# bibendovsky/oalsfxpp

Hardware: AMD Instinct MI355X
Metric: Msamples/sec EAX reverb, 256-frame buffers, batch=4096; % HBM roofline (higher is better)
Workload: dtype f32

## Files before the change

include/oalsfx_hip_debug.h:

```cpp
#ifndef OALSFX_HIP_DEBUG_H
#define OALSFX_HIP_DEBUG_H

#include "oalsfx_hip.h"

#ifdef __cplusplus
extern "C" {
#endif

int oalsfx_batch_mix_timed(oalsfx_batch* b, int frames, const float* src_host, float* dst_host, double legs_us[3]);
long long oalsfx_debug_chain_same_cu(oalsfx_batch* b);
int oalsfx_batch_fill_synthetic(oalsfx_batch* b, int frames, unsigned buffer_index, float* dst_dev, void* hip_stream);

int oalsfx_batch_kernel_timing(oalsfx_batch* b, int enable);
int oalsfx_batch_kernel_timing_read(oalsfx_batch* b, int effect_type, int* launches, double* total_ms);
int oalsfx_batch_kernel_timing_samples(oalsfx_batch* b, int effect_type, double* out_us, int max_samples);
int oalsfx_batch_placement(const oalsfx_batch* b, int* chunks, int* candidates, double* best_us, double* worst_us);
int oalsfx_batch_event_overhead(oalsfx_batch* b, int repeats, double* avg_us);

int oalsfx_debug_hbm_sweep(int device_id, unsigned long long bytes, int write, int repeats);
void oalsfx_debug_set_flags(int flags);
unsigned long long oalsfx_debug_ring_address(oalsfx_batch* b, int instance, int slot);
int oalsfx_debug_move_rings(oalsfx_batch* b, int keep_old);
int oalsfx_debug_probe_rings(oalsfx_batch* b, int repeats, double* avg_us);
int oalsfx_debug_probe_pointer(void* slabs, int instances, int slab_floats, int repeats, double* avg_us);
int oalsfx_debug_stream_pattern(int device_id, int instances, int dwords_per_lane, int repeats, int slab_floats, int pos_skew, double* avg_us);

int oalsfx_debug_host_pipeline(oalsfx_batch* b, int* form, double* probe_us_three_streams, double* probe_us_one_stream);

void oalsfx_debug_gate_skew(oalsfx_batch* b, unsigned skew);
int oalsfx_debug_chain_given_up(const oalsfx_batch* b);
int oalsfx_debug_chain_started(oalsfx_batch* b, unsigned* host_total, unsigned* device_total);
int oalsfx_batch_multi_counts(const oalsfx_batch* b, long long* buffers_in_passes, long long* passes);

long long oalsfx_debug_downmix_uploads(const oalsfx_batch* b);
void oalsfx_debug_downmix_vector(int max_floats);

long long oalsfx_debug_sampler_uploads(const oalsfx_batch* b);
long long oalsfx_debug_envelope_uploads(const oalsfx_batch* b);
const char* oalsfx_debug_last_render_kernel(const oalsfx_batch* b);
long long oalsfx_debug_resampler_uploads(const oalsfx_batch* b);

#ifdef __cplusplus
}
#endif

#endif
```

oalsfxpp_amd/api.py:

```python
import ctypes as C
import operator
import weakref

import numpy as np

from . import desc, lib

_fp = C.POINTER(C.c_float)
DOWNMIX_CHUNK = 32
METER_LANES = 64
METER_CARRY = 1
METER_DTYPE = np.dtype([("peak", np.float32, (desc.MAX_CHANNELS,)), ("sumsq", np.float32, (desc.MAX_CHANNELS,)), ("peak_hold", np.float32),
                        ("quiet_run", np.uint32), ("nonfinite", np.uint32), ("frames", np.uint32)])
assert METER_DTYPE.itemsize == C.sizeof(desc.Meter) == 80
SAMPLER_DTYPE = np.dtype([("data", np.uint64), ("position", np.uint64), ("frames", np.uint32), ("loop_start", np.uint32), ("loop_end", np.uint32),
                          ("step", np.uint32), ("format", np.uint32), ("channels", np.uint32), ("flags", np.uint32), ("reserved", np.uint32),
                          ("gain", np.float32, (desc.MAX_CHANNELS,))])
assert SAMPLER_DTYPE.itemsize == C.sizeof(desc.Sampler) == 80
SAMPLER_FRAC_BITS = desc.SAMPLER_FRAC_BITS
ENVELOPE_DTYPE = np.dtype([("flags", np.uint32), ("delay", np.uint32), ("ramp_frames", np.uint32), ("ramp_done", np.uint32),
                           ("gain_from", np.float32, (desc.MAX_CHANNELS,)), ("gain_step", np.float32, (desc.MAX_CHANNELS,)),
                           ("gain_to", np.float32, (desc.MAX_CHANNELS,)), ("glide_frames", np.uint32), ("glide_done", np.uint32),
                           ("glide_slope", np.int32), ("step_to", np.uint32), ("sub", np.uint32), ("reserved", np.uint32, (3,))])
assert ENVELOPE_DTYPE.itemsize == C.sizeof(desc.Envelope) == 144
# ... 175 lines not shown

    def mix_device(self, frames, src_ptr, dst_ptr, stream=None):
        self._check(self._lib.oalsfx_batch_mix_device(self._h, frames, C.c_void_p(src_ptr), C.c_void_p(dst_ptr), C.c_void_p(stream or 0)))

    def mix_device_multi(self, frames, src_ptrs, dst_ptrs, stream=None):
        if len(src_ptrs) != len(dst_ptrs):
            raise BatchError("mix_device_multi: as many source as destination buffers")
        s = (C.c_void_p * max(1, len(src_ptrs)))(*src_ptrs)
        d = (C.c_void_p * max(1, len(dst_ptrs)))(*dst_ptrs)
        self._check(self._lib.oalsfx_batch_mix_device_multi(self._h, frames, len(src_ptrs), s, d, C.c_void_p(stream or 0)))

    def multi_counts(self):
        k, p = C.c_longlong(0), C.c_longlong(0)
        self._check(self._lib.oalsfx_batch_multi_counts(self._h, C.byref(k), C.byref(p)))
        return k.value, p.value

    def synchronize(self):
        self._check(self._lib.oalsfx_batch_synchronize(self._h))

    @property
    def stream(self):
        return self._lib.oalsfx_batch_stream(self._h)

    def fill_synthetic(self, frames, buffer_index, dst_ptr, stream=None):
        self._check(self._lib.oalsfx_batch_fill_synthetic(self._h, frames, buffer_index, C.c_void_p(dst_ptr), C.c_void_p(stream or 0)))

    def read_slot(self, instance, slot):
        p, s = desc.SlotParams(), desc.SlotState()
        self._check(self._lib.oalsfx_batch_read_slot(self._h, instance, slot, C.byref(p), C.byref(s)))
        return p, s
# ... 586 lines not shown
```

oalsfxpp_amd/csrc/hip/batch.cpp:

```cpp
#include <hip/hip_runtime.h>

#include <algorithm>
#include <atomic>
#include <cstdio>
#include <chrono>
#include <cmath>
#include <cstdlib>
#include <cstring>
#include <map>
#include <mutex>
#include <new>
#include <string>
#include <type_traits>
#include <vector>

#include "../host/core.hpp"
#include "common.hpp"
#include "oalsfx_hip.h"
#include "state_io.hpp"
#include "downmix.hpp"
#include "meter.hpp"
#include "sampler.hpp"
#include "voice.hpp"
#include "resample.hpp"
// ... 145 lines not shown
    uint32_t turn_counter = 0;
    uint32_t started_total = 0;
    int launched_groups = 0;
    uint32_t frames_total = 0;
    std::vector<uint32_t> started_at;
    bool off_grid_known = false;
    int off_grid[OALSFX_MAX_SLOTS] = {};
    bool poisoned = false;
    int chain_len = 0;
    std::vector<std::pair<const char*, const char*>> chain_dsts;
    bool uncached = false;
    bool chain_open = false;
    bool stream_handed_out = false;
    long long chained_calls = 0;
    long long multi_buffers = 0, multi_passes = 0;
    std::vector<int> route_bus;
    std::vector<float> route_gain;
    bool routing_dirty = true;
    int route_max = -1;
    int dm_buses = 0;
    oalsfx_hip::DownmixTable dm_table;
    oalsfx_hip::DownmixDevice dm_dev;
    char* h_dm_table = nullptr;
    char* d_dm_table = nullptr;
    size_t dm_table_capacity = 0;
    float* d_dm_partials = nullptr;
    size_t dm_partials_capacity = 0;
    float* d_dm_out = nullptr;
    size_t dm_out_capacity = 0;
    hipEvent_t ev_downmix = nullptr;
// ... 109 lines not shown
        b->ring_floats[idx] = 0;
    }
}

enum DebugFlag : int {
    kDbgAcquireAlways = 0x1,
    kDbgAcquireNever = 0x2,
    kDbgReadEarly = 0x4,
    kDbgGeneralOnly = 0x8,
    kDbgTapRound128 = 0x20,
    kDbgTapRound256 = 0x40,
    kDbgChainLight = 0x80,
    kDbgNoCuMajor = 0x100,
    kDbgNoChain = 0x400,
    kDbgGateSecondOnly = 0x800,
    kDbgChainAlways = 0x8000,
    kDbgForceProven = 0x2000000,
    kDbgHandOverBits = kDbgAcquireAlways | kDbgAcquireNever | kDbgReadEarly,
    kDbgKernelBits = 0xFF,
};
int debug_flags();

constexpr int kSettleFrames = OALSFX_RV_FADE_SAMPLES;

enum : uint8_t {
    kClassReverb = 1,
    kClassSteady = 2,
    kClassClose = 4,
    kClassShort = 8,
    kClassModulated = 16,
// ... 364 lines not shown
        st.capacity = cap;
    }
    return &st;
}

struct PendingUpload {
    bool any = false;
    oalsfx_batch::Stage* st = nullptr;
    size_t bytes = 0;
    bool direct = true;
    bool chainable = true;
    oalsfx_hip::UploadJobs jobs{};
};

bool chain_join(oalsfx_batch* b);

bool prepare_params(oalsfx_batch* b, PendingUpload& pu)
{
    if (b->dirty_list.empty() && !b->lists_dirty) return true;
    pu.any = true;
    const size_t total = static_cast<size_t>(b->n) * b->slots;
    std::map<size_t, int> need;
    std::vector<size_t> restarted;
    std::vector<int> up_params, up_state, up_source, up_touched;
    std::vector<uint32_t> up_epoch;
    bool any_type_change = false;
    if (!b->dirty_list.empty()) b->upload_gen += 1;

    if (b->last_launch_stream && b->last_launch_stream != b->stream) {
        if (!b->hip_ok(hipStreamWaitEvent(b->stream, b->ev_mixed, 0), "hipStreamWaitEvent")) return false;
// ... 500 lines not shown
    p.use_steady = steady_kernel_usable(ctx);
    p.steady = p.use_steady ? b->fast_count[s] + b->slow_count[s] : 0;
    p.reverbs = b->list_count[s][OALSFX_REVERB] + b->list_count[s][OALSFX_EAX_REVERB];
    p.mixed = p.light > 0 && p.steady > 0 && b->channels <= 2 && !ctx.timeline;
    const int last_block = n - ((n - 1) / OALSFX_RV_MAX_UPDATE) * OALSFX_RV_MAX_UPDATE;
    const bool gains_rest = last_block >= 64 * b->rest_tiles[s];
    p.by_kind = p.use_steady && !p.mixed && b->channels <= 2 && (n & 63) == 0 && !ctx.timeline;
    p.proven_usable = gains_rest;
    p.ragged_proven = p.use_steady && !p.mixed && b->channels <= 2 && (n & 63) != 0 && !ctx.timeline && p.proven_usable && b->slow_count[s] == 0 &&
                      b->fast_count[s] > 0;
    return p;
}

bool chain_join(oalsfx_batch* b)
{
    if (!b->chain_open) return true;
    b->chain_open = false;
    for (int k = 1; k < kChainDepth; ++k) {
        if (!b->chain_used[k]) continue;
        b->chain_used[k] = false;
        if (!b->hip_ok(hipEventRecord(b->ev_chain[k], b->chain_stream[k]), "hipEventRecord") ||
            !b->hip_ok(hipStreamWaitEvent(b->stream, b->ev_chain[k], 0), "hipStreamWaitEvent")) return false;
    }
    return true;
}

bool kernels_serialised_by_a_tool()
{
    static const bool yes = [] {
        const char* on = std::getenv("ROCPROF_COUNTER_COLLECTION");
// ... 10 lines not shown
    if (kernels_serialised_by_a_tool() || b->chain_given_up) return false;
    const size_t buffer_bytes = static_cast<size_t>(b->n) * (frames / buffers) * b->channels * sizeof(float);
    for (int k = 0; k < buffers; ++k) {
        if (reinterpret_cast<uintptr_t>(dsts[k]) % 8 != 0) return false;
        if (b->chain_open && b->chain_dsts.size() >= 256) {
            const char* lo = reinterpret_cast<const char*>(dsts[k]);
            bool known = false;
            for (const auto& d : b->chain_dsts) known |= d.first <= lo && lo < d.second;
            if (!known) return false;
        }
        const char* lo = reinterpret_cast<const char*>(srcs[k]);
        const char* hi = lo + buffer_bytes;
        if (b->chain_open)
            for (const auto& d : b->chain_dsts)
                if (lo < d.second && d.first < hi) return false;
    }
    if (stream != b->stream || b->stream_handed_out || (debug_flags() & (kDbgNoChain | kDbgGeneralOnly)) || b->timing_every > 0 || b->d_timeline) return false;
    if (!b->uncached) return false;
    for (const auto& kv : b->pools)
        if (kv.first % 32 != 0) return false;
    if (frames > OALSFX_MAX_CHUNK) return false;
    if (b->channels > 2) {
        const int last_block = frames - ((frames - 1) / OALSFX_RV_MAX_UPDATE) * OALSFX_RV_MAX_UPDATE;
        return b->slots == 1 && !uploading && (frames & 63) == 0 && b->n_filtered == 0 && b->general_count[0] == 0 && b->slow_count[0] == 0 &&
               b->fast_count[0] == b->n && last_block / 64 >= b->rest_tiles[0];
    }
    if (b->slots > 1) {
        const int last = b->slots - 1, run = reverb_free_run(b, 0);
        if (uploading || (frames & 63) != 0 || b->n_filtered > 0 || run < last) return false;
        if ((b->n + 3) / 4 < 1024 && !(debug_flags() & kDbgChainAlways)) return false;
// ... 22 lines not shown
        ctx.frames = frames;
        if (!plan_slot(b, ctx, 0, frames, true).ragged_proven || b->n_filtered > 0) return false;
    }
    if (b->n_filtered > 0) {
        KernelCtx ctx{};
        ctx.frames = frames;
        const SlotPlan p0 = plan_slot(b, ctx, 0, frames, true);
        if (!p0.by_kind || p0.steady != b->n) return false;
        int counts[4];
        steady_kind_counts(b, 0, p0.proven_usable, counts);
        if (filters_inside_count(b, 0, counts) != b->n_filtered) return false;
    }
    return true;
}

bool chain_next_launch(oalsfx_batch* b, KernelCtx& ctx, int depth, PendingUpload* upload, hipStream_t* stream_out)
{
    b->chain_pos_before = b->chain_open ? b->chain_pos_last : -1;
    b->chain_pos_last = b->chain_open ? b->chain_pos : -1;
    b->chain_pos = b->chain_open ? (b->chain_pos + 1) % depth : 0;
    hipStream_t stream = b->chain_stream[b->chain_pos];
    const bool first_on_its_stream = b->chain_open && !b->chain_used[b->chain_pos];
    b->chain_used[b->chain_pos] = true;
    const size_t total = static_cast<size_t>(b->n) * b->slots;
    ctx.turn = b->d_turn;
    ctx.turn_cu = b->d_turn + total + 16;
    ctx.turn_cu2 = ctx.turn_cu + total;
    ctx.turn_slot = b->slots - 1;
    ctx.turn_two_back = (b->chain_pos_before >= 0 && b->chain_pos_before != b->chain_pos) ? 1u : 0u;
    ctx.turn_wait = b->chain_open ? b->turn_counter : 0u;
    if (++b->turn_counter == 0u) b->turn_counter = 1u;
    ctx.turn_set = b->turn_counter;
    unsigned* started = b->d_turn + total;
    if (!b->chain_open) {
        if (!b->hip_ok(hipEventRecord(b->ev_chain_start, b->stream), "hipEventRecord")) return false;
        b->chain_len = 1;
    } else {
        ++b->chain_len;
        if (first_on_its_stream && !b->hip_ok(hipStreamWaitEvent(stream, b->ev_chain_start, 0), "hipStreamWaitEvent")) return false;
        if (b->chain_len == 2 || !(debug_flags() & kDbgGateSecondOnly)) {
            const unsigned target = b->started_total - static_cast<uint32_t>(std::min(8, (b->n + 3) / 4 - 1));
            if (upload && upload->st) { upload->jobs.gate_started = started; upload->jobs.gate_target = target + b->gate_skew; }
            else oalsfx_hip::launch_chain_gate(started, target + b->gate_skew, b->d_fault + 1, stream);
        }
    }
    ctx.turn_started = started;
    b->chain_open = true;
    b->launched_groups = 0;
    *stream_out = stream;
    return true;
}

bool chain_launch_done(oalsfx_batch* b)
{
    if (b->launched_groups <= 0) return b->fail("Internal error: a chained call launched no grid that takes turns.");
    b->started_total += static_cast<uint32_t>(b->launched_groups);
    b->launched_groups = 0;
    return true;
}

// ... 22 lines not shown
        r.push_back({reinterpret_cast<uintptr_t>(srcs[k]), k, false});
        r.push_back({reinterpret_cast<uintptr_t>(dsts[k]), k, true});
    }
    std::sort(r.begin(), r.end(), [](const Range& x, const Range& y) { return x.lo < y.lo || (x.lo == y.lo && x.call < y.call); });
    const Range* last[2][2] = {};
    for (const Range& x : r) {
        for (int kind = 0; kind < 2; ++kind) {
            if (!x.out && kind == 0) continue;
            for (const Range* y : last[kind])
                if (y && y->call != x.call && y->lo + bytes > x.lo) return false;
        }
        const int kind = x.out ? 1 : 0;
        last[kind][1] = last[kind][0];
        last[kind][0] = &x;
    }
    return true;
}

bool mix_pass(oalsfx_batch* b, int frames, int buffers, const float* const* srcs, float* const* dsts, hipStream_t stream, bool may_chain,
              PendingUpload& upload, bool pass)
{
    const float* const src = srcs[0];
    float* const dst = dsts[0];
    const int total = frames * buffers;
    if (pass && total > OALSFX_MAX_CHUNK) return b->fail("Internal error: a multi-buffer pass longer than one chunk.");
    const bool chained = may_chain && (!upload.st || upload.chainable) && chain_eligible(b, total, buffers, srcs, dsts, stream, upload.st != nullptr);
    if (!chained && !chain_join(b)) return false;
    int depth = 2;
    if (chained) {
        const int rs = b->slots - 1;
// ... 20 lines not shown
    }
    KernelCtx ctx{};
    ctx.params = b->d_params;
    ctx.state = b->d_state;
    ctx.rings = b->d_rings;
    ctx.source = b->d_source;
    ctx.source_state = b->d_source_state;
    ctx.mixbuf = b->d_mixbuf;
    ctx.timeline = b->d_timeline;
    ctx.hot = b->d_hot;
    ctx.inst_epoch = b->d_inst_epoch;
    ctx.exact = b->d_exact;
    ctx.fault = b->d_fault;
    ctx.list_first = -1;
    ctx.no_follow_up = 0;
    if (chained) {
        if (!b->chain_open) b->chain_dsts.clear();
        for (int k = 0; k < buffers; ++k) {
            const char* lo = reinterpret_cast<const char*>(dsts[k]);
            const char* hi = lo + static_cast<size_t>(b->n) * frames * b->channels * sizeof(float);
            bool known = false;
            for (auto& d : b->chain_dsts) known |= d.first <= lo && hi <= d.second;
            if (!known) b->chain_dsts.push_back({lo, hi});
        }
        if (!chain_next_launch(b, ctx, depth, &upload, &stream)) return false;
        if (!launch_params(b, upload, stream, nullptr, b->d_turn, ctx.turn_wait)) return false;
        b->chained_calls += 1;
    }
    ctx.slots = b->slots;
    ctx.channels = b->channels;
    ctx.io_stride = static_cast<long long>(frames) * b->channels;
    struct EqualPlaces {
        bool on;
        explicit EqualPlaces(bool o) : on(o) { if (on) oalsfx_hip::set_lds_per_workgroup(40960); }
        ~EqualPlaces() { if (on) oalsfx_hip::set_lds_per_workgroup(0); }
    } equal_places(chained && b->slots > 1);
    oalsfx_hip::BufferTable table{};
    if (pass) {
        for (int k = 0; k < buffers; ++k) { table.src[k] = srcs[k]; table.dst[k] = dsts[k]; }
        table.frames = frames;
// ... 69 lines not shown
            int main_part = -1;
            for (int g = 0; g < 4; ++g)
                if (part_on[g]) main_part = (main_part < 0 || g == 3) ? g : main_part;
            int side = 0;
            for (int g = 0; g < 4; ++g) {
                if (!part_on[g]) continue;
                hipStream_t gs = stream;
                if (fork && g != main_part) {
                    gs = b->side_stream[side];
                    if (!b->hip_ok(hipStreamWaitEvent(gs, b->ev_fork, 0), "hipStreamWaitEvent")) return false;
                }
                if (g == 0) {
                    launch_wave_group(b, ctx, s, flags, gs);
                } else if (g == 2 && mixed) {
                    launch_mixed_part(b, ctx, s, flags, gs);
                } else if (g == 2 && pass) {
                    launch_reverb_pass_part(b, ctx, s, flags, table, gs);
                } else if (g == 2 && by_kind) {
                    launch_reverb_kinds_part(b, ctx, s, flags, proven_usable, filters_inside, gs);
                } else if (g == 2) {
                    launch_reverb_steady_part(b, ctx, s, flags, b->steady_offset[s], steady, sp.ragged_proven, gs);
                } else {
                    launch_reverb_general_part(b, !use_steady, ctx, s, flags, gs);
                }
                if (gs != stream) {
                    if (!b->hip_ok(hipEventRecord(b->ev_join[side], gs), "hipEventRecord")) return false;
                    ++side;
                }
            }
            for (int k = 0; k < side; ++k)
// ... 28 lines not shown
{
    if (b->state_io_unordered && stream != b->stream) {
        if (!b->hip_ok(hipStreamWaitEvent(stream, b->ev_state_io, 0), "hipStreamWaitEvent")) return false;
        b->state_io_unordered = false;
    }
    const int per_pass = std::max(1, OALSFX_MAX_CHUNK / std::max(frames, 1));
    const bool apart = multi && buffers_apart(b, frames, buffers, srcs, dsts);
    for (int k = 0; k < buffers;) {
        if (b->poisoned) return b->fail(b->fault_text);
        poll_exact(b);
        b->launched_groups = 0;
        PendingUpload upload;
        const auto hp0 = std::chrono::steady_clock::now();
        if (!prepare_params(b, upload)) return false;
        b->host_prepare_ns += std::chrono::duration_cast<std::chrono::nanoseconds>(std::chrono::steady_clock::now() - hp0).count();
        const int take = std::min(buffers - k, per_pass);
        const bool pass = apart && !(debug_flags() & kDbgGeneralOnly) && pass_usable(b, frames, take * frames);
        const int step = pass ? take : 1;
        if (!mix_pass(b, frames, step, srcs + k, dsts + k, stream, may_chain, upload, pass)) return false;
        k += step;
    }
    return true;
}

bool mix_device(oalsfx_batch* b, int frames, const float* src, float* dst, hipStream_t stream, bool may_chain = false)
{
    float* out = dst;
    return mix_device(b, frames, 1, &src, &out, stream, may_chain, false);
}

// ... 127 lines not shown
        ok = b->hip_ok(hipMalloc(reinterpret_cast<void**>(&b->d_timeline), kTimelineBytes), "hipMalloc(timeline)");
        ok = ok && b->hip_ok(hipMemsetAsync(b->d_timeline, 0, kTimelineBytes, b->stream), "hipMemsetAsync(timeline)");
    }
    if (!ok) {
        g_last_error = b->error;
        oalsfx_batch_destroy(b);
        return nullptr;
    }
    return b;
}

void oalsfx_batch_destroy(oalsfx_batch* b)
{
    if (!b) return;
    hipSetDevice(b->device);
    for (int k = 1; k < kChainDepth; ++k)
        if (b->chain_stream[k]) hipStreamSynchronize(b->chain_stream[k]);
    if (b->stream) hipStreamSynchronize(b->stream);
    for (int k = 0; k < kSideStreams; ++k)
        if (b->side_stream[k]) hipStreamSynchronize(b->side_stream[k]);
    if (b->exact_pending) hipEventSynchronize(b->ev_exact);
    if (b->d_timeline) {
        std::vector<unsigned long long> h(kTimelineBytes / sizeof(unsigned long long));
        if (hipMemcpy(h.data(), b->d_timeline, kTimelineBytes, hipMemcpyDeviceToHost) == hipSuccess)
            if (FILE* f = std::fopen(std::getenv("OALSFX_DEBUG_TIMELINE"), "wb")) { std::fwrite(h.data(), 1, kTimelineBytes, f); std::fclose(f); }
        hipFree(b->d_timeline);
    }
    for (auto& t : b->timed) { hipEventDestroy(t.start); hipEventDestroy(t.stop); }
    for (hipEvent_t e : b->event_pool) hipEventDestroy(e);
    if (std::getenv("OALSFX_HOST_PROFILE"))
// ... 10 lines not shown
        if (b->chain_stream[k]) hipStreamDestroy(b->chain_stream[k]);
    if (b->h2d_stream) hipStreamSynchronize(b->h2d_stream);
    if (b->d2h_stream) hipStreamSynchronize(b->d2h_stream);
    for (auto& ps : b->pipe) {
        hipFree(ps.d_src); hipFree(ps.d_dst);
        if (ps.copied_in) hipEventDestroy(ps.copied_in);
        if (ps.mixed) hipEventDestroy(ps.mixed);
        if (ps.copied_out) hipEventDestroy(ps.copied_out);
    }
    if (b->h2d_stream) hipStreamDestroy(b->h2d_stream);
    if (b->d2h_stream) hipStreamDestroy(b->d2h_stream);
    if (b->h_io_src) (void)hipHostFree(b->h_io_src);
    if (b->h_io_dst) (void)hipHostFree(b->h_io_dst);
    if (b->h_exact) (void)hipHostFree(b->h_exact);
    if (b->h_fault) (void)hipHostFree(b->h_fault);
    if (b->ev_exact) hipEventDestroy(b->ev_exact);
    if (b->h_state_io) (void)hipHostFree(b->h_state_io);
    hipFree(b->d_state_io);
    if (b->ev_state_io) hipEventDestroy(b->ev_state_io);
    if (b->dm_pending) hipEventSynchronize(b->ev_downmix);
    if (b->h_dm_table) (void)hipHostFree(b->h_dm_table);
    hipFree(b->d_dm_table); hipFree(b->d_dm_partials); hipFree(b->d_dm_out);
    hipFree(b->d_meters);
    if (b->sampler_pending) hipEventSynchronize(b->ev_sampler);
    if (b->h_sampler_stage) (void)hipHostFree(b->h_sampler_stage);
    hipFree(b->d_samplers);
    if (b->ev_sampler) hipEventDestroy(b->ev_sampler);
    if (b->ev_sampler_staged) hipEventDestroy(b->ev_sampler_staged);
    if (b->h_envelope_stage) (void)hipHostFree(b->h_envelope_stage);
    hipFree(b->d_envelopes);
// ... 1564 lines not shown
    return 1;
}

const char* oalsfx_batch_last_reverb_kernel(const oalsfx_batch* b) { return b->last_steady_kernel; }

long long oalsfx_batch_chained_calls(const oalsfx_batch* b) { return b->chained_calls; }

int oalsfx_batch_multi_counts(const oalsfx_batch* b, long long* buffers_in_passes, long long* passes)
{
    if (!b) { g_last_error = "Null batch."; return 0; }
    if (buffers_in_passes) *buffers_in_passes = b->multi_buffers;
    if (passes) *passes = b->multi_passes;
    return 1;
}

long long oalsfx_debug_chain_same_cu(oalsfx_batch* b)
{
    unsigned v = 0;
    if (hipSetDevice(b->device) != hipSuccess || !chain_join(b) || hipStreamSynchronize(b->stream) != hipSuccess) return -1;
    if (hipMemcpy(&v, b->d_turn + static_cast<size_t>(b->n) * b->slots + 1, sizeof(v), hipMemcpyDeviceToHost) != hipSuccess) return -1;
    return v;
}

int oalsfx_debug_host_pipeline(oalsfx_batch* b, int* form, double* probe_us_three_streams, double* probe_us_one_stream)
{
    if (form) *form = b->pipe_mode;
    if (probe_us_three_streams) *probe_us_three_streams = b->pipe_probe_us[0];
    if (probe_us_one_stream) *probe_us_one_stream = b->pipe_probe_us[1];
    return 1;
}
// ... 176 lines not shown
```

oalsfxpp_amd/csrc/hip/common.hpp:

```cpp
#ifndef OALSFX_HIP_COMMON_HPP
#define OALSFX_HIP_COMMON_HPP

#include <hip/hip_runtime.h>
#include <stdint.h>

#include "oalsfx_desc.h"

namespace oalsfx_hip {

struct alignas(128) SlotStateLines : oalsfx_slot_state {};
static_assert(sizeof(SlotStateLines) % 128 == 0 && sizeof(oalsfx_source_state) % 128 == 0, "an instance's records end where its cache lines end");


struct KernelCtx {
    const oalsfx_slot_params* params;
    SlotStateLines* state;
    float* const* rings;
    const oalsfx_source_params* source;
    oalsfx_source_state* source_state;
    const float* raw_src;
    const float* src;
    const float* wet_src;
    long long wet_plane;
    float* dst;
// ... 59 lines not shown
constexpr unsigned kPlainMinTapAhead = 224;

const char* launch_reverb_steady(const KernelCtx& ctx, int slot, const int* list, int count, int flags, bool close_taps, bool modulated,
                                 bool short_taps, bool proven, bool in_transition, hipStream_t stream, int* groups = nullptr, bool carry = false);
const char* launch_reverb_steady_kinds(const KernelCtx& ctx, int slot, const int* list, const int counts[4], int flags, bool filters_inside,
                                       hipStream_t stream, int* groups = nullptr, bool carry = false);
constexpr int kMaxPassBuffers = 32;
struct BufferTable {
    const float* src[kMaxPassBuffers];
    float* dst[kMaxPassBuffers];
    int frames;
    int buffers;
};
const char* launch_reverb_steady_multi(const KernelCtx& ctx, int slot, const int* list, const int counts[3], const BufferTable& table, int flags,
                                       hipStream_t stream, int* groups = nullptr, bool carry = false);
void launch_reverb_general(const KernelCtx& ctx, int slot, const int* list, int count, int flags, hipStream_t stream);
void launch_wave_effects(const KernelCtx& ctx, int slot, int slot_count, const int* list, int count, const WaveSegments* seg, int flags,
                         hipStream_t stream);
void launch_slot_mixed(const KernelCtx& ctx, int slot, const int* steady_list, int steady_count, const int* light_list, int light_count,
                       const WaveSegments& seg, int flags, bool proven, hipStream_t stream, int* groups = nullptr);
constexpr unsigned kFaultTurn = 1u << 12;
constexpr unsigned kFaultGate = 1u << 24;

void launch_chain_gate(const unsigned* started, unsigned target, unsigned* fault, hipStream_t stream);
void launch_send_filters(const KernelCtx& ctx, const float* src, long long src_stride, float* filtered, size_t send_floats, const int* list, int instances,
                         hipStream_t stream);
void launch_scatter_records(void* dst, size_t record_bytes, const void* packed, const int* indices, int count, hipStream_t stream);
struct ScatterJob { unsigned* dst; const unsigned* packed; const int* indices; int record_dwords; int count; int takes_turns; };
struct CopyJob { unsigned* dst; const unsigned* src; size_t dwords; int blocks; };
struct UploadJobs { ScatterJob scatter[4]; CopyJob copy[2]; const unsigned* turn; unsigned turn_wait; unsigned* fault; const unsigned* gate_started; unsigned gate_target; };
void launch_upload(UploadJobs jobs, hipStream_t stream);
void launch_null(hipStream_t stream);
void launch_fill_synthetic(float* dst, int instances, int floats_per_instance, unsigned buffer_index, hipStream_t stream);
void launch_ring_probe(float* slabs, int instances, size_t slab_floats, unsigned pos0, int waves_per_slab, hipStream_t stream);
void launch_stream_pattern(float* slabs, int instances, int dwords_per_lane, unsigned pos0, size_t slab_floats, int pos_skew, hipStream_t stream);
void launch_hbm_sweep(float* buf, size_t floats, int write, float* sink, hipStream_t stream);

void set_lds_per_workgroup(int bytes);
int lds_per_workgroup();
// ... 196 lines not shown
```

oalsfxpp_amd/csrc/hip/reverb.hip:

```cpp
#include <float.h>

#include "common.hpp"
#include "wave_effects_body.hpp"

namespace oalsfx_hip {

namespace {

constexpr int kRow = 68;
constexpr int kGroups = 3;
constexpr int kSteadyGroups = 6;
constexpr int kRngFloats = OALSFX_RV_MAX_UPDATE;

namespace ut {
enum {
    TAP4 = 0,
    LO = 24,
    BMASK = 44,
    FEED4 = 49,
    CR_R = 50, CR_RF = 51,
    ECOEF = 52, ELCOEF = 56,
    MISC = 60,
    LPB = 64, HPB = 68,
    TL0 = 72, TL1 = 76, TH0 = 80, TH1 = 84,
// ... 1555 lines not shown
    if (group < kinds.groups(0)) {
        reverb_steady_group<CH, 4, false, false, false, false, false, true, false, false, false, CR, true>(ctx, slot, list, kinds.count[0], flags, group, sh.lean, &table);
        return;
    }
    group -= kinds.groups(0);
    list += kinds.count[0];
    if (group < kinds.groups(1)) {
        reverb_steady_group<CH, 4, false, true, false, false, false, true, false, false, false, 0, true>(ctx, slot, list, kinds.count[1], flags, group, sh.lean, &table);
        return;
    }
    group -= kinds.groups(1);
    list += kinds.count[1];
    reverb_steady_group<CH, 4, false, true, true, true, false, true, false, false, false, 0, true>(ctx, slot, list, kinds.count[2], flags, group, sh.general, &table);
}

template <int CH>
__device__ __forceinline__ void reverb_general_instance(const KernelCtx& ctx, int slot, int inst, int flags, float* lds, int lane)
{
    constexpr int NQ = Lds<CH>::kChains;
    auto row = [&](int group, int c) -> float* { return lds + (group * 4 + c) * kRow; };
    float* rng = lds + kGroups * 4 * kRow;
    float* gseq = rng + kRngFloats;
    float* utf = gseq + NQ * 64;
    unsigned* utu = reinterpret_cast<unsigned*>(utf);

    int gts_i = 0;
    auto gstamp = [&]() {
        if (ctx.timeline && (inst & 63) == 0 && (inst >> 6) < 64 && lane == 0 && gts_i < 96)
            ctx.timeline[64 * 4 * 96 + (inst >> 6) * 96 + gts_i++] = clock64();
    };
// ... 746 lines not shown
#define OALSFX_MULTI(...)                                                                                          \
    do {                                                                                                           \
        OALSFX_LAUNCH((k_reverb_steady_multi<__VA_ARGS__>), grid, block, stream, c, slot, list, kinds, flags, table); \
        return "k_reverb_steady_multi<" #__VA_ARGS__ ">";                                                          \
    } while (0)
    const bool carry_all = carry && counts[0] > 0;
    if (c.channels == 1) {
        if (carry_all) OALSFX_MULTI(1, 2);
        OALSFX_MULTI(1, 0);
    }
    if (carry_all) OALSFX_MULTI(2, 2);
    OALSFX_MULTI(2, 0);
#undef OALSFX_MULTI
}

void launch_reverb_general(const KernelCtx& ctx, int slot, const int* list, int count, int flags, hipStream_t stream)
{
    if (count <= 0) return;
    const dim3 grid((count + 3) / 4), block(256);
    const KernelCtx& c = ctx;
    if (c.channels == 1) OALSFX_LAUNCH(k_reverb<1>, grid, block, stream, c, slot, list, count, flags);
    else if (c.channels == 2) OALSFX_LAUNCH(k_reverb<2>, grid, block, stream, c, slot, list, count, flags);
    else OALSFX_LAUNCH(k_reverb<8>, grid, block, stream, c, slot, list, count, flags);
}

}
```

oalsfxpp_amd/csrc/hip/support_kernels.hip:

```cpp
#include <algorithm>

#include "common.hpp"

namespace oalsfx_hip {

namespace { thread_local int t_lds_per_workgroup = 0; }
void set_lds_per_workgroup(int bytes) { t_lds_per_workgroup = bytes; }
int lds_per_workgroup() { return t_lds_per_workgroup; }

namespace {
constexpr int kFilterRow = 4 + 64;
constexpr int kFilterRowsPerWave = 48;
constexpr int kFilterInstances = 2;
constexpr int kFilterTable = kFilterInstances * 5 * 8;

inline __host__ __device__ int filter_instances_per_wave(int channels, int slots)
{
    const int chains = (1 + slots) * channels, rows = channels + chains;
    int n = 64 / chains;
    if (n > kFilterRowsPerWave / rows) n = kFilterRowsPerWave / rows;
    return n < 1 ? 1 : (n > kFilterInstances ? kFilterInstances : n);
}

__device__ __forceinline__ void filter_recurrence(float* row, int n, float a1, float a2, float& y1, float& y2)
// ... 200 lines not shown
__device__ __forceinline__ void chain_gate_wait(const unsigned* started, unsigned target, unsigned* fault)
{
    unsigned* gave_up = const_cast<unsigned*>(started) + 2;
    if (__hip_atomic_load(gave_up, __ATOMIC_RELAXED, __HIP_MEMORY_SCOPE_AGENT) != 0u) return;
    unsigned spins = 0;
    while (static_cast<int>(__hip_atomic_load(started, __ATOMIC_RELAXED, __HIP_MEMORY_SCOPE_AGENT) - target) < 0) {
        __builtin_amdgcn_s_sleep(8);
        if (++spins > (1u << 22)) {
            if (fault) __hip_atomic_fetch_add(fault, kFaultGate, __ATOMIC_RELAXED, __HIP_MEMORY_SCOPE_SYSTEM);
            __hip_atomic_store(gave_up, 1u, __ATOMIC_RELAXED, __HIP_MEMORY_SCOPE_AGENT);
            break;
        }
    }
}

__global__ __launch_bounds__(64) void k_chain_gate(const unsigned* started, unsigned target, unsigned* fault)
{
    if (threadIdx.x == 0) chain_gate_wait(started, target, fault);
}

void launch_chain_gate(const unsigned* started, unsigned target, unsigned* fault, hipStream_t stream)
{
    hipLaunchKernelGGL(k_chain_gate, dim3(1), dim3(64), 0, stream, started, target, fault);
}

void launch_send_filters(const KernelCtx& ctx, const float* src, long long src_stride, float* filtered, size_t send_floats, const int* list, int instances,
                         hipStream_t stream)
{
    if (instances <= 0 || ctx.frames <= 0) return;
    const int ipw = filter_instances_per_wave(ctx.channels, ctx.slots);
    const int waves = (instances + ipw - 1) / ipw;
    hipLaunchKernelGGL(k_send_filters, dim3((waves + 3) / 4), dim3(256), 0, stream, ctx, src, src_stride, filtered, send_floats, list, instances);
}

__global__ void k_fill_synthetic(float* dst, int instances, int floats_per_instance, unsigned buffer_index)
{
    const int inst = blockIdx.x * blockDim.x + threadIdx.x;
    if (inst >= instances) return;
// ... 203 lines not shown
```

oalsfxpp_amd/lib.py:

```python
import ctypes as C
import os

from . import desc

_HERE = os.path.dirname(os.path.abspath(__file__))
LIB_PATH = os.path.join(_HERE, "csrc", "liboalsfx_hip.so")

_fp = C.POINTER(C.c_float)
_lib = None

SIGNATURES = {
    "oalsfx_batch_create": (C.c_void_p, [C.c_int, C.c_int, C.c_int, C.c_int, C.c_int]),
    "oalsfx_batch_destroy": (None, [C.c_void_p]),
    "oalsfx_batch_error": (C.c_char_p, [C.c_void_p]),
    "oalsfx_last_error": (C.c_char_p, []),
    "oalsfx_batch_instances": (C.c_int, [C.c_void_p]),
    "oalsfx_batch_channels": (C.c_int, [C.c_void_p]),
    "oalsfx_batch_sampling_rate": (C.c_int, [C.c_void_p]),
    "oalsfx_batch_effect_count": (C.c_int, [C.c_void_p]),
    "oalsfx_batch_set_effect": (C.c_int, [C.c_void_p, C.c_int, C.c_int, C.c_int, C.c_void_p, C.c_int]),
    "oalsfx_batch_set_effect_at": (C.c_int, [C.c_void_p, C.c_void_p, C.c_int, C.c_int, C.c_void_p, C.c_int]),
    "oalsfx_batch_set_effect_type": (C.c_int, [C.c_void_p, C.c_int, C.c_int, C.c_int, C.c_int]),
    "oalsfx_batch_set_effect_props": (C.c_int, [C.c_void_p, C.c_int, C.c_int, C.c_int, C.c_void_p, C.c_int]),
    "oalsfx_batch_set_send_props": (C.c_int, [C.c_void_p, C.c_int, C.c_int, C.c_int, C.POINTER(desc.SendProps)]),
# ... 57 lines not shown
    "oalsfx_group_set_effect_props": (C.c_int, [C.c_void_p, C.c_int, C.c_int, C.c_int, C.c_void_p, C.c_int]),
    "oalsfx_group_set_send_props": (C.c_int, [C.c_void_p, C.c_int, C.c_int, C.c_int, C.POINTER(desc.SendProps)]),
    "oalsfx_group_apply_changes": (C.c_int, [C.c_void_p, C.c_int, C.c_int]),
    "oalsfx_group_mix": (C.c_int, [C.c_void_p, C.c_int, C.c_void_p, C.c_void_p]),
    "oalsfx_group_mix_device": (C.c_int, [C.c_void_p, C.c_int, C.POINTER(C.c_void_p), C.POINTER(C.c_void_p)]),
    "oalsfx_group_mix_device_multi": (C.c_int, [C.c_void_p, C.c_int, C.c_int, C.POINTER(C.c_void_p), C.POINTER(C.c_void_p)]),
    "oalsfx_group_set_routing": (C.c_int, [C.c_void_p, C.c_int, C.c_int, C.POINTER(C.c_int), _fp]),
    "oalsfx_group_mix_downmix": (C.c_int, [C.c_void_p, C.c_int, _fp, C.c_int, _fp]),
    "oalsfx_group_mix_downmix_meter": (C.c_int, [C.c_void_p, C.c_int, _fp, C.c_int, _fp, C.c_float, C.c_int, C.c_void_p]),
    "oalsfx_group_synchronize": (C.c_int, [C.c_void_p]),
    "oalsfx_trim_pools": (C.c_ulonglong, []),
    "oalsfx_pools_waiting_bytes": (C.c_ulonglong, []),
    "oalsfx_debug_chain_same_cu": (C.c_longlong, [C.c_void_p]),
    "oalsfx_debug_chain_started": (C.c_int, [C.c_void_p, C.POINTER(C.c_uint), C.POINTER(C.c_uint)]),
    "oalsfx_batch_multi_counts": (C.c_int, [C.c_void_p, C.POINTER(C.c_longlong), C.POINTER(C.c_longlong)]),
    "oalsfx_debug_downmix_uploads": (C.c_longlong, [C.c_void_p]),
    "oalsfx_debug_downmix_vector": (None, [C.c_int]),
    "oalsfx_debug_sampler_uploads": (C.c_longlong, [C.c_void_p]),
    "oalsfx_debug_envelope_uploads": (C.c_longlong, [C.c_void_p]),
    "oalsfx_debug_resampler_uploads": (C.c_longlong, [C.c_void_p]),
    "oalsfx_debug_last_render_kernel": (C.c_char_p, [C.c_void_p]),
    "oalsfx_debug_gate_skew": (None, [C.c_void_p, C.c_uint]),
    "oalsfx_debug_chain_given_up": (C.c_int, [C.c_void_p]),
    "oalsfx_debug_host_pipeline": (C.c_int, [C.c_void_p, C.POINTER(C.c_int), C.POINTER(C.c_double), C.POINTER(C.c_double)]),
    "oalsfx_device_pci_bus_id": (C.c_int, [C.c_int, C.c_char_p, C.c_int]),
    "oalsfx_debug_set_flags": (None, [C.c_int]),
    "oalsfx_debug_ring_address": (C.c_ulonglong, [C.c_void_p, C.c_int, C.c_int]),
    "oalsfx_debug_move_rings": (C.c_int, [C.c_void_p, C.c_int]),
    "oalsfx_debug_probe_rings": (C.c_int, [C.c_void_p, C.c_int, C.POINTER(C.c_double)]),
    "oalsfx_debug_probe_pointer": (C.c_int, [C.c_void_p, C.c_int, C.c_int, C.c_int, C.POINTER(C.c_double)]),
# ... 83 lines not shown
```

Before: 25530.

## Join consecutive chained mix calls into one reverb launch via host-mapped slot

```diff
diff --git a/include/oalsfx_hip_debug.h b/include/oalsfx_hip_debug.h
--- a/include/oalsfx_hip_debug.h
+++ b/include/oalsfx_hip_debug.h
@@ -32,6 +32,10 @@
 int oalsfx_debug_chain_started(oalsfx_batch* b, unsigned* host_total, unsigned* device_total);
 int oalsfx_batch_multi_counts(const oalsfx_batch* b, long long* buffers_in_passes, long long* passes);
 
+int oalsfx_batch_join_counts(const oalsfx_batch* b, long long* joined_calls, long long* joinable_launches);
+#define OALSFX_DEBUG_NO_JOIN 0x1000
+void oalsfx_debug_join_hold(oalsfx_batch* b, int k);
+
 long long oalsfx_debug_downmix_uploads(const oalsfx_batch* b);
 void oalsfx_debug_downmix_vector(int max_floats);
 
diff --git a/oalsfxpp_amd/api.py b/oalsfxpp_amd/api.py
--- a/oalsfxpp_amd/api.py
+++ b/oalsfxpp_amd/api.py
@@ -213,6 +213,14 @@
         k, p = C.c_longlong(0), C.c_longlong(0)
         self._check(self._lib.oalsfx_batch_multi_counts(self._h, C.byref(k), C.byref(p)))
         return k.value, p.value
+
+    def join_counts(self):
+        j, l = C.c_longlong(0), C.c_longlong(0)
+        self._check(self._lib.oalsfx_batch_join_counts(self._h, C.byref(j), C.byref(l)))
+        return j.value, l.value
+
+    def join_hold(self, k):
+        self._lib.oalsfx_debug_join_hold(self._h, int(k))
 
     def synchronize(self):
         self._check(self._lib.oalsfx_batch_synchronize(self._h))
diff --git a/oalsfxpp_amd/csrc/hip/batch.cpp b/oalsfxpp_amd/csrc/hip/batch.cpp
--- a/oalsfxpp_amd/csrc/hip/batch.cpp
+++ b/oalsfxpp_amd/csrc/hip/batch.cpp
@@ -183,6 +183,31 @@
     bool stream_handed_out = false;
     long long chained_calls = 0;
     long long multi_buffers = 0, multi_passes = 0;
+    static constexpr int kJoinSlots = 1024;
+    oalsfx_join::JoinSlot* h_join = nullptr;
+    oalsfx_join::JoinSlot* d_join = nullptr;
+    oalsfx_hip::BufferTable* d_join_tables = nullptr;
+    int join_turn = 0;
+    struct JoinLaunch {
+        bool accepting = false;
+        bool held = false;
+        int slot = 0, table = 0;
+        unsigned count = 0;
+        int frames = 0;
+        KernelCtx ctx{};
+        hipStream_t stream = nullptr;
+        int reverb_slot = 0, flags = 0;
+        const int* list = nullptr;
+        int counts[4] = {};
+        int groups = 0;
+        bool carry = false;
+        const unsigned* gate_started = nullptr;
+        unsigned gate_target = 0;
+        const char* srcs[oalsfx_join::kMaxBuffers] = {};
+        const char* dsts[oalsfx_join::kMaxBuffers] = {};
+    } join;
+    int join_hold = 0;
+    long long joined_calls = 0, joinable_launches = 0;
     std::vector<int> route_bus;
     std::vector<float> route_gain;
     bool routing_dirty = true;
@@ -322,6 +347,7 @@
     kDbgNoCuMajor = 0x100,
     kDbgNoChain = 0x400,
     kDbgGateSecondOnly = 0x800,
+    kDbgNoJoin = OALSFX_DEBUG_NO_JOIN,
     kDbgChainAlways = 0x8000,
     kDbgForceProven = 0x2000000,
     kDbgHandOverBits = kDbgAcquireAlways | kDbgAcquireNever | kDbgReadEarly,
@@ -716,6 +742,7 @@
 };
 
 bool chain_join(oalsfx_batch* b);
+void join_flush(oalsfx_batch* b);
 
 bool prepare_params(oalsfx_batch* b, PendingUpload& pu)
 {
@@ -1246,6 +1273,7 @@
 
 bool chain_join(oalsfx_batch* b)
 {
+    join_flush(b);
     if (!b->chain_open) return true;
     b->chain_open = false;
     for (int k = 1; k < kChainDepth; ++k) {
@@ -1286,6 +1314,10 @@
         if (b->chain_open)
             for (const auto& d : b->chain_dsts)
                 if (lo < d.second && d.first < hi) return false;
+        const char* out_lo = reinterpret_cast<const char*>(dsts[k]);
+        if (b->chain_open)
+            for (const auto& d : b->chain_dsts)
+                if (out_lo != d.first && out_lo < d.second && d.first < out_lo + buffer_bytes) return false;
     }
     if (stream != b->stream || b->stream_handed_out || (debug_flags() & (kDbgNoChain | kDbgGeneralOnly)) || b->timing_every > 0 || b->d_timeline) return false;
     if (!b->uncached) return false;
@@ -1338,8 +1370,9 @@
     return true;
 }
 
-bool chain_next_launch(oalsfx_batch* b, KernelCtx& ctx, int depth, PendingUpload* upload, hipStream_t* stream_out)
-{
+bool chain_next_launch(oalsfx_batch* b, KernelCtx& ctx, int depth, PendingUpload* upload, hipStream_t* stream_out, bool* joinable = nullptr)
+{
+    bool own_gate = false;
     b->chain_pos_before = b->chain_open ? b->chain_pos_last : -1;
     b->chain_pos_last = b->chain_open ? b->chain_pos : -1;
     b->chain_pos = b->chain_open ? (b->chain_pos + 1) % depth : 0;
@@ -1365,9 +1398,11 @@
         if (b->chain_len == 2 || !(debug_flags() & kDbgGateSecondOnly)) {
             const unsigned target = b->started_total - static_cast<uint32_t>(std::min(8, (b->n + 3) / 4 - 1));
             if (upload && upload->st) { upload->jobs.gate_started = started; upload->jobs.gate_target = target + b->gate_skew; }
+            else if (joinable && *joinable) { own_gate = true; b->join.gate_started = started; b->join.gate_target = target + b->gate_skew; b->join.table = b->chain_pos; }
             else oalsfx_hip::launch_chain_gate(started, target + b->gate_skew, b->d_fault + 1, stream);
         }
     }
+    if (joinable) *joinable = own_gate;
     ctx.turn_started = started;
     b->chain_open = true;
     b->launched_groups = 0;
@@ -1420,6 +1455,122 @@
         last[kind][1] = last[kind][0];
         last[kind][0] = &x;
     }
+    return true;
+}
+
+bool join_atomics(int device)
+{
+    static std::mutex m;
+    static std::map<int, bool> known;
+    std::lock_guard<std::mutex> lock(m);
+    auto it = known.find(device);
+    if (it != known.end()) return it->second;
+    int v = 0;
+    const bool ok = hipDeviceGetAttribute(&v, hipDeviceAttributeHostNativeAtomicSupported, device) == hipSuccess && v != 0;
+    if (!ok) std::fprintf(stderr, "oalsfx: device %d reports no native atomics on host memory: queued launches take no later calls (chained launches as before).\n", device);
+    known[device] = ok;
+    return ok;
+}
+
+void join_queue(oalsfx_batch* b)
+{
+    auto& j = b->join;
+    if (!j.held) return;
+    j.held = false;
+    oalsfx_hip::launch_chain_gate(j.gate_started, j.gate_target, b->d_fault + 1, j.stream, b->d_join + j.slot, b->d_join_tables + j.table, static_cast<unsigned>(j.groups));
+    const char* name = oalsfx_hip::launch_reverb_steady_joined(j.ctx, j.reverb_slot, j.list, j.counts, b->d_join_tables + j.table, j.flags, j.stream, nullptr, j.carry);
+    if (name) b->last_steady_kernel = name;
+}
+
+void join_flush(oalsfx_batch* b)
+{
+    b->join.accepting = false;
+    join_queue(b);
+}
+
+bool join_wanted(oalsfx_batch* b, int frames)
+{
+    if ((debug_flags() & (kDbgNoJoin | kDbgGateSecondOnly)) || frames > OALSFX_MAX_CHUNK || b->exact_wanted) return false;
+    if (!pass_usable(b, frames, frames) || !join_atomics(b->device)) return false;
+    if (!b->h_join) {
+        if (hipHostMalloc(reinterpret_cast<void**>(&b->h_join), oalsfx_batch::kJoinSlots * sizeof(oalsfx_join::JoinSlot), hipHostMallocMapped) != hipSuccess) { b->h_join = nullptr; return false; }
+        std::memset(b->h_join, 0, oalsfx_batch::kJoinSlots * sizeof(oalsfx_join::JoinSlot));
+        if (hipHostGetDevicePointer(reinterpret_cast<void**>(&b->d_join), b->h_join, 0) != hipSuccess ||
+            handed_on_malloc(b, reinterpret_cast<void**>(&b->d_join_tables), kChainDepth * sizeof(oalsfx_hip::BufferTable)) != hipSuccess) {
+            (void)hipHostFree(b->h_join);
+            b->h_join = nullptr;
+            (void)hipGetLastError();
+            return false;
+        }
+    }
+    if (!b->d_join_tables) return false;
+    return oalsfx_join::join_reusable(b->h_join + b->join_turn);
+}
+
+bool join_begin(oalsfx_batch* b, const KernelCtx& ctx, int slot, int flags, const float* src, float* dst, hipStream_t stream)
+{
+    auto& j = b->join;
+    j.slot = b->join_turn;
+    b->join_turn = (b->join_turn + 1) % oalsfx_batch::kJoinSlots;
+    j.count = 1;
+    j.frames = ctx.frames;
+    j.ctx = ctx;
+    j.stream = stream;
+    j.reverb_slot = slot;
+    j.flags = flags | ((debug_flags() & kDbgKernelBits) << 8) | ((debug_flags() & kDbgNoCuMajor) ? oalsfx_hip::kNoCuMajor : 0);
+    j.list = b->d_lists + b->steady_offset[slot];
+    steady_kind_counts(b, slot, true, j.counts);
+    j.carry = slot_off_grid(b, slot);
+    j.srcs[0] = reinterpret_cast<const char*>(src);
+    j.dsts[0] = reinterpret_cast<const char*>(dst);
+    int groups = 0;
+    for (int k = 0; k < 3; ++k) groups += (j.counts[k] + 3) >> 2;
+    if (groups <= 0) return b->fail("Internal error: a joinable launch without instances.");
+    b->launched_groups += groups;
+    j.groups = groups;
+    oalsfx_join::join_start(b->h_join + j.slot, j.frames, src, dst);
+    j.accepting = j.frames * 2 <= OALSFX_MAX_CHUNK;
+    j.held = true;
+    b->joinable_launches += 1;
+    if (b->join_hold <= 1 || !j.accepting) join_queue(b);
+    return true;
+}
+
+bool join_try(oalsfx_batch* b, int frames, const float* src, float* dst, hipStream_t stream, const PendingUpload& upload)
+{
+    auto& j = b->join;
+    if (!j.accepting) return false;
+    if (!b->chain_open || stream != b->stream || frames != j.frames || upload.st || upload.any || b->exact_wanted || (debug_flags() & kDbgNoJoin)) return false;
+    const int total = static_cast<int>(j.count + 1) * frames;
+    if (total > OALSFX_MAX_CHUNK || !pass_usable(b, frames, total)) return false;
+    float* out = dst;
+    if (!chain_eligible(b, frames, 1, &src, &out, stream, false)) return false;
+    const size_t bytes = static_cast<size_t>(b->n) * frames * b->channels * sizeof(float);
+    const char* lo = reinterpret_cast<const char*>(dst);
+    const char* in = reinterpret_cast<const char*>(src);
+    for (unsigned k = 0; k < j.count; ++k) {
+        if (lo != j.dsts[k] && lo < j.dsts[k] + bytes && j.dsts[k] < lo + bytes) return false;
+        if (lo < j.srcs[k] + bytes && j.srcs[k] < lo + bytes) return false;
+    }
+    if (in != lo && in < lo + bytes && lo < in + bytes) return false;
+    if (!oalsfx_join::join_append(b->h_join + j.slot, j.count, src, dst)) { j.accepting = false; return false; }
+    j.srcs[j.count] = in;
+    j.dsts[j.count] = lo;
+    j.count += 1;
+    b->mix_calls += 1;
+    b->chained_calls += 1;
+    b->joined_calls += 1;
+    b->started_total += static_cast<uint32_t>(j.groups);
+    {
+        bool known = false;
+        for (auto& d : b->chain_dsts) known |= d.first <= lo && lo + bytes <= d.second;
+        if (!known) b->chain_dsts.push_back({lo, lo + bytes});
+    }
+    advance_settling(b, frames);
+    b->frames_total += static_cast<uint32_t>(frames);
+    b->last_launch_stream = b->stream;
+    if (static_cast<int>(j.count + 1) * frames > OALSFX_MAX_CHUNK) j.accepting = false;
+    if (j.held && (static_cast<int>(j.count) >= b->join_hold || !j.accepting)) join_flush(b);
     return true;
 }
 
@@ -1470,6 +1621,7 @@
     ctx.fault = b->d_fault;
     ctx.list_first = -1;
     ctx.no_follow_up = 0;
+    bool joinable = false;
     if (chained) {
         if (!b->chain_open) b->chain_dsts.clear();
         for (int k = 0; k < buffers; ++k) {
@@ -1479,7 +1631,8 @@
             for (auto& d : b->chain_dsts) known |= d.first <= lo && hi <= d.second;
             if (!known) b->chain_dsts.push_back({lo, hi});
         }
-        if (!chain_next_launch(b, ctx, depth, &upload, &stream)) return false;
+        joinable = !pass && b->chain_open && b->chain_len >= 2 && !upload.st && join_wanted(b, frames);
+        if (!chain_next_launch(b, ctx, depth, &upload, &stream, &joinable)) return false;
         if (!launch_params(b, upload, stream, nullptr, b->d_turn, ctx.turn_wait)) return false;
         b->chained_calls += 1;
     }
@@ -1579,6 +1732,8 @@
                     launch_wave_group(b, ctx, s, flags, gs);
                 } else if (g == 2 && mixed) {
                     launch_mixed_part(b, ctx, s, flags, gs);
+                } else if (g == 2 && joinable) {
+                    if (!join_begin(b, ctx, s, flags, src, dst, gs)) return false;
                 } else if (g == 2 && pass) {
                     launch_reverb_pass_part(b, ctx, s, flags, table, gs);
                 } else if (g == 2 && by_kind) {
@@ -1637,6 +1792,8 @@
         const auto hp0 = std::chrono::steady_clock::now();
         if (!prepare_params(b, upload)) return false;
         b->host_prepare_ns += std::chrono::duration_cast<std::chrono::nanoseconds>(std::chrono::steady_clock::now() - hp0).count();
+        if (buffers == 1 && !multi && may_chain && join_try(b, frames, srcs[k], dsts[k], stream, upload)) return true;
+        join_flush(b);
         const int take = std::min(buffers - k, per_pass);
         const bool pass = apart && !(debug_flags() & kDbgGeneralOnly) && pass_usable(b, frames, take * frames);
         const int step = pass ? take : 1;
@@ -1794,6 +1951,7 @@
 {
     if (!b) return;
     hipSetDevice(b->device);
+    join_flush(b);
     for (int k = 1; k < kChainDepth; ++k)
         if (b->chain_stream[k]) hipStreamSynchronize(b->chain_stream[k]);
     if (b->stream) hipStreamSynchronize(b->stream);
@@ -1834,6 +1992,8 @@
     if (b->h_io_dst) (void)hipHostFree(b->h_io_dst);
     if (b->h_exact) (void)hipHostFree(b->h_exact);
     if (b->h_fault) (void)hipHostFree(b->h_fault);
+    if (b->h_join) (void)hipHostFree(b->h_join);
+    handed_on_free(b->d_join_tables);
     if (b->ev_exact) hipEventDestroy(b->ev_exact);
     if (b->h_state_io) (void)hipHostFree(b->h_state_io);
     hipFree(b->d_state_io);
@@ -3428,6 +3588,21 @@
     return 1;
 }
 
+int oalsfx_batch_join_counts(const oalsfx_batch* b, long long* joined_calls, long long* joinable_launches)
+{
+    if (!b) { g_last_error = "Null batch."; return 0; }
+    if (joined_calls) *joined_calls = b->joined_calls;
+    if (joinable_launches) *joinable_launches = b->joinable_launches;
+    return 1;
+}
+
+void oalsfx_debug_join_hold(oalsfx_batch* b, int k)
+{
+    if (!b) return;
+    b->join_hold = k;
+    if (k <= 1 && hipSetDevice(b->device) == hipSuccess) join_queue(b);
+}
+
 long long oalsfx_debug_chain_same_cu(oalsfx_batch* b)
 {
     unsigned v = 0;
diff --git a/oalsfxpp_amd/csrc/hip/common.hpp b/oalsfxpp_amd/csrc/hip/common.hpp
--- a/oalsfxpp_amd/csrc/hip/common.hpp
+++ b/oalsfxpp_amd/csrc/hip/common.hpp
@@ -2,9 +2,11 @@
 #define OALSFX_HIP_COMMON_HPP
 
 #include <hip/hip_runtime.h>
+#include <stddef.h>
 #include <stdint.h>
 
 #include "oalsfx_desc.h"
+#include "join_word.hpp"
 
 namespace oalsfx_hip {
 
@@ -97,6 +99,11 @@
 };
 const char* launch_reverb_steady_multi(const KernelCtx& ctx, int slot, const int* list, const int counts[3], const BufferTable& table, int flags,
                                        hipStream_t stream, int* groups = nullptr, bool carry = false);
+static_assert(sizeof(BufferTable) == sizeof(oalsfx_join::JoinTable) && offsetof(BufferTable, dst) == offsetof(oalsfx_join::JoinTable, dst) &&
+              offsetof(BufferTable, frames) == offsetof(oalsfx_join::JoinTable, frames) && offsetof(BufferTable, buffers) == offsetof(oalsfx_join::JoinTable, buffers) &&
+              kMaxPassBuffers == oalsfx_join::kMaxBuffers, "the gate writes a JoinTable where the grid reads a BufferTable");
+const char* launch_reverb_steady_joined(const KernelCtx& ctx, int slot, const int* list, const int counts[3], const BufferTable* table, int flags,
+                                        hipStream_t stream, int* groups = nullptr, bool carry = false);
 void launch_reverb_general(const KernelCtx& ctx, int slot, const int* list, int count, int flags, hipStream_t stream);
 void launch_wave_effects(const KernelCtx& ctx, int slot, int slot_count, const int* list, int count, const WaveSegments* seg, int flags,
                          hipStream_t stream);
@@ -105,7 +112,8 @@
 constexpr unsigned kFaultTurn = 1u << 12;
 constexpr unsigned kFaultGate = 1u << 24;
 
-void launch_chain_gate(const unsigned* started, unsigned target, unsigned* fault, hipStream_t stream);
+void launch_chain_gate(const unsigned* started, unsigned target, unsigned* fault, hipStream_t stream, void* join_slot = nullptr, void* join_table = nullptr,
+                       unsigned join_groups = 0);
 void launch_send_filters(const KernelCtx& ctx, const float* src, long long src_stride, float* filtered, size_t send_floats, const int* list, int instances,
                          hipStream_t stream);
 void launch_scatter_records(void* dst, size_t record_bytes, const void* packed, const int* indices, int count, hipStream_t stream);
diff --git a/oalsfxpp_amd/csrc/hip/join_word.hpp b/oalsfxpp_amd/csrc/hip/join_word.hpp
--- /dev/null
+++ b/oalsfxpp_amd/csrc/hip/join_word.hpp
@@ -0,0 +1,80 @@
+#ifndef OALSFX_JOIN_WORD_HPP
+#define OALSFX_JOIN_WORD_HPP
+
+#include <cstdint>
+
+#if defined(__HIPCC__)
+#define OALSFX_JOIN_FN __host__ __device__ inline
+#else
+#define OALSFX_JOIN_FN inline
+#endif
+
+namespace oalsfx_join {
+
+constexpr int kMaxBuffers = 32;
+constexpr uint64_t kJoinOpen = 1ull << 63, kJoinClosed = 1ull << 62, kJoinDone = 1ull << 61, kJoinCountMask = 0xFFFFFFFFull;
+
+struct JoinTable {
+    const float* src[kMaxBuffers];
+    float* dst[kMaxBuffers];
+    int frames;
+    int buffers;
+};
+
+struct JoinSlot {
+    uint64_t word;
+    int frames;
+    int pad;
+    const float* src[kMaxBuffers];
+    float* dst[kMaxBuffers];
+};
+
+OALSFX_JOIN_FN bool join_reusable(const JoinSlot* s)
+{
+    const uint64_t w = __atomic_load_n(&s->word, __ATOMIC_ACQUIRE);
+    return w == 0 || (w & kJoinDone) != 0;
+}
+
+OALSFX_JOIN_FN void join_start(JoinSlot* s, int frames, const float* src, float* dst)
+{
+    s->frames = frames;
+    s->src[0] = src;
+    s->dst[0] = dst;
+    __atomic_store_n(&s->word, kJoinOpen | 1u, __ATOMIC_RELEASE);
+}
+
+OALSFX_JOIN_FN bool join_append(JoinSlot* s, unsigned count, const float* src, float* dst)
+{
+    if (count >= static_cast<unsigned>(kMaxBuffers)) return false;
+    s->src[count] = src;
+    s->dst[count] = dst;
+    uint64_t expected = kJoinOpen | count;
+    return __atomic_compare_exchange_n(&s->word, &expected, kJoinOpen | (count + 1u), false, __ATOMIC_RELEASE, __ATOMIC_RELAXED);
+}
+
+OALSFX_JOIN_FN unsigned join_close(JoinSlot* s)
+{
+    const uint64_t old = __atomic_exchange_n(&s->word, kJoinClosed, __ATOMIC_ACQUIRE);
+    return (old & kJoinOpen) ? static_cast<unsigned>(old & kJoinCountMask) : 0u;
+}
+
+OALSFX_JOIN_FN void join_copy_entry(const JoinSlot* s, JoinTable* t, unsigned k)
+{
+    t->src[k] = s->src[k];
+    t->dst[k] = s->dst[k];
+}
+
+OALSFX_JOIN_FN void join_copy_sizes(const JoinSlot* s, JoinTable* t, unsigned count)
+{
+    t->frames = s->frames;
+    t->buffers = static_cast<int>(count);
+}
+
+OALSFX_JOIN_FN void join_done(JoinSlot* s, unsigned count)
+{
+    __atomic_store_n(&s->word, kJoinDone | count, __ATOMIC_RELEASE);
+}
+
+}
+
+#endif
diff --git a/oalsfxpp_amd/csrc/hip/reverb.hip b/oalsfxpp_amd/csrc/hip/reverb.hip
--- a/oalsfxpp_amd/csrc/hip/reverb.hip
+++ b/oalsfxpp_amd/csrc/hip/reverb.hip
@@ -1593,6 +1593,32 @@
     reverb_steady_group<CH, 4, false, true, true, true, false, true, false, false, false, 0, true>(ctx, slot, list, kinds.count[2], flags, group, sh.general, &table);
 }
 
+template <int CH, int CR>
+__global__ __launch_bounds__(256, 4) void k_reverb_steady_joined(KernelCtx ctx, int slot, const int* __restrict__ list, SteadyKinds kinds, int flags, const BufferTable* __restrict__ table)
+{
+    union Shared {
+        SteadyShared<CH, 4, true, false, false, false, CR> lean;
+        SteadyShared<CH, 4, true, true, true> general;
+    };
+    __shared__ Shared sh;
+    KernelCtx c = ctx;
+    c.frames = __builtin_amdgcn_readfirstlane(table->frames * table->buffers);
+    int group = (flags & kNoCuMajor) ? static_cast<int>(blockIdx.x) : cu_major_position(static_cast<int>(blockIdx.x), static_cast<int>(gridDim.x));
+    if (group < kinds.groups(0)) {
+        reverb_steady_group<CH, 4, false, false, false, false, false, true, false, false, false, CR, true>(c, slot, list, kinds.count[0], flags, group, sh.lean, table);
+        return;
+    }
+    group -= kinds.groups(0);
+    list += kinds.count[0];
+    if (group < kinds.groups(1)) {
+        reverb_steady_group<CH, 4, false, true, false, false, false, true, false, false, false, 0, true>(c, slot, list, kinds.count[1], flags, group, sh.lean, table);
+        return;
+    }
+    group -= kinds.groups(1);
+    list += kinds.count[1];
+    reverb_steady_group<CH, 4, false, true, true, true, false, true, false, false, false, 0, true>(c, slot, list, kinds.count[2], flags, group, sh.general, table);
+}
+
 template <int CH>
 __device__ __forceinline__ void reverb_general_instance(const KernelCtx& ctx, int slot, int inst, int flags, float* lds, int lane)
 {
@@ -2369,6 +2395,32 @@
 #undef OALSFX_MULTI
 }
 
+const char* launch_reverb_steady_joined(const KernelCtx& ctx, int slot, const int* list, const int counts[3], const BufferTable* table, int flags,
+                                        hipStream_t stream, int* groups_out, bool carry)
+{
+    KernelCtx c = ctx;
+    c.list_first = -1;
+    SteadyKinds kinds{};
+    int groups = 0;
+    for (int k = 0; k < 3; ++k) { kinds.count[k] = counts[k]; groups += kinds.groups(k); }
+    if (groups_out) *groups_out = groups;
+    if (groups <= 0) return nullptr;
+    const dim3 grid(groups), block(256);
+#define OALSFX_JOINED(...)                                                                                          \
+    do {                                                                                                            \
+        OALSFX_LAUNCH((k_reverb_steady_joined<__VA_ARGS__>), grid, block, stream, c, slot, list, kinds, flags, table); \
+        return "k_reverb_steady_joined<" #__VA_ARGS__ ">";                                                          \
+    } while (0)
+    const bool carry_all = carry && counts[0] > 0;
+    if (c.channels == 1) {
+        if (carry_all) OALSFX_JOINED(1, 2);
+        OALSFX_JOINED(1, 0);
+    }
+    if (carry_all) OALSFX_JOINED(2, 2);
+    OALSFX_JOINED(2, 0);
+#undef OALSFX_JOINED
+}
+
 void launch_reverb_general(const KernelCtx& ctx, int slot, const int* list, int count, int flags, hipStream_t stream)
 {
     if (count <= 0) return;
diff --git a/oalsfxpp_amd/csrc/hip/support_kernels.hip b/oalsfxpp_amd/csrc/hip/support_kernels.hip
--- a/oalsfxpp_amd/csrc/hip/support_kernels.hip
+++ b/oalsfxpp_amd/csrc/hip/support_kernels.hip
@@ -238,14 +238,26 @@
     }
 }
 
-__global__ __launch_bounds__(64) void k_chain_gate(const unsigned* started, unsigned target, unsigned* fault)
+__global__ __launch_bounds__(64) void k_chain_gate(const unsigned* started, unsigned target, unsigned* fault, oalsfx_join::JoinSlot* join, oalsfx_join::JoinTable* table,
+                                                   unsigned groups)
 {
     if (threadIdx.x == 0) chain_gate_wait(started, target, fault);
-}
-
-void launch_chain_gate(const unsigned* started, unsigned target, unsigned* fault, hipStream_t stream)
-{
-    hipLaunchKernelGGL(k_chain_gate, dim3(1), dim3(64), 0, stream, started, target, fault);
+    if (join == nullptr) return;
+    unsigned count = 0;
+    if (threadIdx.x == 0) count = oalsfx_join::join_close(join);
+    count = static_cast<unsigned>(__builtin_amdgcn_readfirstlane(static_cast<int>(count)));
+    if (count > static_cast<unsigned>(oalsfx_join::kMaxBuffers)) count = oalsfx_join::kMaxBuffers;
+    if (threadIdx.x < count) oalsfx_join::join_copy_entry(join, table, threadIdx.x);
+    if (threadIdx.x == 0) oalsfx_join::join_copy_sizes(join, table, count);
+    if (threadIdx.x == 0 && count > 1u) __hip_atomic_fetch_add(const_cast<unsigned*>(started), (count - 1u) * groups, __ATOMIC_RELAXED, __HIP_MEMORY_SCOPE_AGENT);
+    __builtin_amdgcn_fence(__ATOMIC_RELEASE, "");
+    if (threadIdx.x == 0) oalsfx_join::join_done(join, count);
+}
+
+void launch_chain_gate(const unsigned* started, unsigned target, unsigned* fault, hipStream_t stream, void* join_slot, void* join_table, unsigned join_groups)
+{
+    hipLaunchKernelGGL(k_chain_gate, dim3(1), dim3(64), 0, stream, started, target, fault, static_cast<oalsfx_join::JoinSlot*>(join_slot),
+                       static_cast<oalsfx_join::JoinTable*>(join_table), join_groups);
 }
 
 void launch_send_filters(const KernelCtx& ctx, const float* src, long long src_stride, float* filtered, size_t send_floats, const int* list, int instances,
diff --git a/oalsfxpp_amd/lib.py b/oalsfxpp_amd/lib.py
--- a/oalsfxpp_amd/lib.py
+++ b/oalsfxpp_amd/lib.py
@@ -95,6 +95,8 @@
     "oalsfx_debug_chain_same_cu": (C.c_longlong, [C.c_void_p]),
     "oalsfx_debug_chain_started": (C.c_int, [C.c_void_p, C.POINTER(C.c_uint), C.POINTER(C.c_uint)]),
     "oalsfx_batch_multi_counts": (C.c_int, [C.c_void_p, C.POINTER(C.c_longlong), C.POINTER(C.c_longlong)]),
+    "oalsfx_batch_join_counts": (C.c_int, [C.c_void_p, C.POINTER(C.c_longlong), C.POINTER(C.c_longlong)]),
+    "oalsfx_debug_join_hold": (None, [C.c_void_p, C.c_int]),
     "oalsfx_debug_downmix_uploads": (C.c_longlong, [C.c_void_p]),
     "oalsfx_debug_downmix_vector": (None, [C.c_int]),
     "oalsfx_debug_sampler_uploads": (C.c_longlong, [C.c_void_p]),
```

After: 28510, median of 6. +11.7%, better.
